# ZPP-Robotics/OSQP-Solver

Measured on AMD Instinct MI355X. Metric: QPs/sec on a 1024-QP batch of box-QPs (n=512, m=1024), OSQP defaults; ADMM iters/sec alongside, higher is better.
Workload: dtype f64

## Files before the change

### include/mi_osqp.h

```cpp
#ifndef MI_OSQP_H
#define MI_OSQP_H

#include <stdint.h>

#ifdef __cplusplus
extern "C" {
#endif

typedef enum {
  MI_OSQP_OK = 0,
  MI_OSQP_ERR_INVALID_DATA = 1,
  MI_OSQP_ERR_INVALID_SETTINGS = 2,
  MI_OSQP_ERR_PATTERN_CHANGED = 3,
  MI_OSQP_ERR_NONCONVEX = 4,
  MI_OSQP_ERR_DEVICE = 5,
  MI_OSQP_ERR_NULL = 6,
  MI_OSQP_ERR_ALLOC = 7
} mi_osqp_error;

typedef enum {
  MI_OSQP_EXIT_OPTIMAL = 0,
  MI_OSQP_EXIT_PRIMAL_INFEASIBLE = 1,
  MI_OSQP_EXIT_DUAL_INFEASIBLE = 2,
  MI_OSQP_EXIT_OPTIMAL_INACCURATE = 3,
// ... 112 lines not shown
                                  const double *l, const double *u);
int mi_osqp_batch_warm_start_x(mi_osqp_batch *h, const double *x);
int mi_osqp_batch_update_q(mi_osqp_batch *h, const double *q);
int mi_osqp_batch_update_P(mi_osqp_batch *h, const int64_t *P_colptr, const int64_t *P_rowidx, const double *P_val);
int mi_osqp_batch_update_P_A(mi_osqp_batch *h, const int64_t *P_colptr, const int64_t *P_rowidx, const double *P_val,
                             const int64_t *A_colptr, const int64_t *A_rowidx, const double *A_val);
int mi_osqp_batch_warm_start_y(mi_osqp_batch *h, const double *y);
int mi_osqp_batch_get_P_upper_pattern(mi_osqp_batch *h, int64_t *colptr, int64_t *rowidx, int64_t *nnz_out);
int mi_osqp_batch_solve(mi_osqp_batch *h);
int mi_osqp_batch_get_primal(mi_osqp_batch *h, double *x_out );
int mi_osqp_batch_get_dual(mi_osqp_batch *h, double *y_out );
int mi_osqp_batch_get_info(mi_osqp_batch *h, mi_osqp_info *info );
int mi_osqp_batch_get_prim_inf_cert(mi_osqp_batch *h, double *dy_out );
int mi_osqp_batch_get_dual_inf_cert(mi_osqp_batch *h, double *dx_out );
int mi_osqp_batch_get_stats(mi_osqp_batch *h, mi_osqp_stats *st);
int mi_osqp_batch_get_ordering(mi_osqp_batch *h, int64_t *kkt_perm);
void mi_osqp_batch_free(mi_osqp_batch *h);
int mi_osqp_prefetch_analysis(int64_t B, int64_t n, int64_t m, const int64_t *Pp, const int64_t *Pi,
                              const int64_t *Ap, const int64_t *Ai, int64_t device);
void mi_osqp_release_device_cache(void);

int mi_osqp_batch_update_bounds_device(mi_osqp_batch *h, const double *d_l, const double *d_u, void *stream);
int mi_osqp_batch_update_A_bounds_device(mi_osqp_batch *h, const double *d_Av, const double *d_l, const double *d_u, void *stream);
int mi_osqp_batch_update_q_device(mi_osqp_batch *h, const double *d_q, void *stream);
int mi_osqp_batch_update_P_device(mi_osqp_batch *h, const double *d_Pv, void *stream);
int mi_osqp_batch_update_P_A_bounds_device(mi_osqp_batch *h, const double *d_Pv, const double *d_Av, const double *d_l, const double *d_u,
                                           void *stream);
int mi_osqp_batch_solve_device(mi_osqp_batch *h, double *d_x_out, int32_t *d_status, int32_t *d_iters, void *stream);
int mi_osqp_batch_reset(mi_osqp_batch *h);
int mi_osqp_batch_last_solve_stats(mi_osqp_batch *h, int64_t *total_iters, int64_t *kernel_launches,
// ... 184 lines not shown
```

### osqp-solver_amd/__init__.py

```python
import ctypes as C
import os

import numpy as np

try:
    import torch
except ImportError:
    torch = None

from . import build as _build

_HERE = os.path.dirname(os.path.abspath(__file__))
_LIB = None

EXIT_NAMES = ["kOptimal", "kPrimalInfeasible", "kDualInfeasible", "kOptimalInaccurate",
              "kPrimalInfeasibleInaccurate", "kDualInfeasibleInaccurate", "kMaxIterations",
              "kInterrupted", "kTimeLimitReached", "kNonConvex", "kUnknown"]
K_OPTIMAL = 0


class Settings(C.Structure):
    _fields_ = [("rho", C.c_double), ("sigma", C.c_double), ("scaling", C.c_int64),
                ("adaptive_rho", C.c_int64), ("adaptive_rho_interval", C.c_int64),
                ("adaptive_rho_tolerance", C.c_double), ("max_iter", C.c_int64),
# ... 88 lines not shown
        L.mi_osqp_get_settings.argtypes = [vp, C.POINTER(Settings)]
        L.mi_osqp_update_settings.argtypes = [vp, C.POINTER(Settings)]
        L.mi_osqp_multi_batch_get_settings.argtypes = [vp, C.POINTER(Settings)]
        L.mi_osqp_multi_batch_update_settings.argtypes = [vp, C.POINTER(Settings)]
        L.mi_osqp_multi_batch_update_rho_each.argtypes = [vp, dp]
        L.mi_osqp_batch_solve.argtypes = [vp]
        L.mi_osqp_batch_get_primal.argtypes = [vp, dp]
        L.mi_osqp_batch_get_dual.argtypes = [vp, dp]
        L.mi_osqp_batch_get_info.argtypes = [vp, C.POINTER(Info)]
        for f in ("mi_osqp_get_prim_inf_cert", "mi_osqp_get_dual_inf_cert", "mi_osqp_batch_get_prim_inf_cert",
                  "mi_osqp_batch_get_dual_inf_cert", "mi_osqp_multi_batch_get_prim_inf_cert", "mi_osqp_multi_batch_get_dual_inf_cert"):
            getattr(L, f).argtypes = [vp, dp]
        L.mi_osqp_batch_get_prim_inf_cert_some.argtypes = [vp, C.c_int64, ip, dp]
        L.mi_osqp_batch_get_dual_inf_cert_some.argtypes = [vp, C.c_int64, ip, dp]
        L.mi_osqp_batch_get_stats.argtypes = [vp, C.POINTER(Stats)]
        L.mi_osqp_batch_get_ordering.argtypes = [vp, ip]
        L.mi_osqp_batch_free.argtypes = [vp]; L.mi_osqp_batch_free.restype = None
        L.mi_osqp_batch_update_bounds_device.argtypes = [vp, vp, vp, vp]
        L.mi_osqp_batch_update_A_bounds_device.argtypes = [vp, vp, vp, vp, vp]
        L.mi_osqp_batch_solve_device.argtypes = [vp, vp, vp, vp, vp]
        L.mi_osqp_batch_reset.argtypes = [vp]
        L.mi_osqp_batch_refactor_device.argtypes = [vp]
        L.mi_osqp_batch_last_solve_stats.argtypes = [vp, ip, ip, dp, dp, ip, dp]
        L.mi_osqp_batch_last_polish_stats.argtypes = [vp, ip, ip, dp]
        L.mi_osqp_batch_get_polish_active.argtypes = [vp, C.POINTER(C.c_int8)]
        L.mi_osqp_batch_adjoint.argtypes = [vp, dp, dp, dp, dp, dp, dp, dp, C.POINTER(C.c_int32)]
        L.mi_osqp_adjoint.argtypes = [vp, dp, dp, dp, dp, dp, dp, dp, C.POINTER(C.c_int32)]
        L.mi_osqp_batch_adjoint_device.argtypes = [vp] * 10
        L.mi_osqp_batch_get_scaling.argtypes = [vp, dp, dp, dp]
        L.mi_osqp_batch_spmv.argtypes = [vp, vp, vp, vp, vp, vp, vp]
# ... 212 lines not shown
    def prim_inf_cert(self):
        v = np.empty((self.B, self.m))
        _chk(lib().mi_osqp_batch_get_prim_inf_cert(self._h, _dp(v)), "get_prim_inf_cert")
        return v

    def dual_inf_cert(self):
        v = np.empty((self.B, self.n))
        _chk(lib().mi_osqp_batch_get_dual_inf_cert(self._h, _dp(v)), "get_dual_inf_cert")
        return v

    def stats(self):
        s = Stats()
        _chk(lib().mi_osqp_batch_get_stats(self._h, C.byref(s)), "get_stats")
        return s.as_dict()

    def ordering(self):
        perm = np.empty(self.n + self.m, dtype=np.int64)
        _chk(lib().mi_osqp_batch_get_ordering(self._h, _ip(perm)), "get_ordering")
        return perm

    def update_A(self, Ax, A_pattern=None):
        Ax = _f64(Ax).reshape(self.B, -1)
        Ap, Ai = self._Ap, self._Ai
        if A_pattern is not None:
            A = _csc(A_pattern)
            Ap, Ai = _i64(A.indptr), _i64(A.indices)
            if len(Ai) != len(self._Ai):
                raise MiOsqpError(3, "update_A")
        _chk(lib().mi_osqp_batch_update_A(self._h, _ip(Ap), _ip(Ai), _dp(Ax)), "update_A")

# ... 522 lines not shown
```

### osqp-solver_amd/csrc/device_types.h

```cpp
#pragma once
#include <hip/hip_runtime.h>
#include <stdint.h>

namespace miosqp {

#define MI_CHUNK 16

struct SchedDev {
  const uint32_t *step, *idxw;
  const uint64_t *idxw64;
  const uint32_t *lvl_pos, *tail_bar;
  int n_phases, nw, n_levels;
  uint32_t n_steps, n_slots;
};

struct DenseTailDev {
  int s, k, n_phases;
  uint32_t n_steps;
  const uint32_t *task;
  const uint32_t *wave_task, *wave_step, *tail_bar;
};

enum { DS_C = 0, DS_CINV, DS_RHO, DS_RHO_EST, DS_PRI_RES, DS_DUA_RES, DS_OBJ, DS_COUNT };
enum { IS_STATUS = 0, IS_ITER, IS_RHO_UPDATES, IS_DONE, IS_NEED_REFACTOR, IS_CUR, IS_PENDING, IS_EPOCH, IS_COUNT };
// ... 26 lines not shown
  int wide;
  double sigma, alpha, eps_abs, eps_rel, eps_prim_inf, eps_dual_inf, rho_tolerance;
  int check_termination, rho_interval, max_iter, scaled_termination, scaling, adaptive_rho;
  int iter_begin, iter_end;
  int op_out_lds;
  int info_at_end;
  int mw_groups;
  unsigned *mw_bar;
  double *mw_scratch;
  int df;
  unsigned df_shadow;
  const unsigned char *rflag;
  const int *sel;
  const int *tiles;
  double *res;
};

struct FactorArgs {
  int n, m, N, B, nnzP, nnzK, pa_len, n_levels, force_all;
  int debug_skip;
  uint32_t storage;
  SchedDev fwd, bwd;
  const uint32_t *blk, *lvl, *utask, *tri4, *dtask, *ttask, *asm_dst, *asm_src;
  const uint32_t *ubig;
  int *use_work;
  const int32_t *fwd_srcblk, *bwd_srcblk;
  const double *pa_val, *l, *u, *dscal;
  double *rho_vec, *rho_inv, *Lblk, *Dl, *dinv_scratch, *fwd_val, *bwd_val, *dinv;
  int *iscal, *npos;
  int home_bt;
// ... 163 lines not shown
```

### osqp-solver_amd/csrc/host_core.cpp

```cpp
#include "host_core.hpp"
#include "sched_format.h"

#include <algorithm>
#include <cmath>
#include <cstdio>
#include <cstdlib>
#include <cstring>
#include <limits>
#include <numeric>
#include <set>
#include <chrono>
#include <thread>

#include "../../include/mi_osqp.h"

namespace miosqp {

int validate_settings(const Settings &s) {
  if (s.scaling < 0 || s.max_iter <= 0 || s.check_termination < 0) return 1;
  if (s.adaptive_rho != 0 && s.adaptive_rho != 1) return 1;
  if (s.adaptive_rho_interval < 0 || s.adaptive_rho_tolerance < 1.0) return 1;
  if (!(s.rho > 0.0) || !(s.sigma > 0.0)) return 1;
  if (s.eps_abs < 0.0 || s.eps_rel < 0.0 || (s.eps_abs == 0.0 && s.eps_rel == 0.0)) return 1;
  if (!(s.eps_prim_inf > 0.0) || !(s.eps_dual_inf > 0.0)) return 1;
// ... 920 lines not shown
  t.stream_factor = getenv("MI_OSQP_STREAM_FACTOR") != nullptr;
  if (const char *e = getenv("MI_OSQP_REFACTOR_PIPELINE")) t.refactor_pipeline = atoi(e) != 0;
  if (const char *e = getenv("MI_OSQP_REFACTOR_PIPELINE_MIN")) t.pipeline_min = std::max(0, atoi(e));
  if (const char *e = getenv("MI_OSQP_REFACTOR_CHUNKS")) t.pipeline_chunks = std::max(0, std::min(8, atoi(e)));
  if (const char *e = getenv("MI_OSQP_REFACTOR_CHUNK_QPS")) t.pipeline_chunk_qps = std::max(0, atoi(e));
  if (const char *e = getenv("MI_OSQP_REFACTOR_LANES")) t.refactor_lanes = std::max(1, std::min(3, atoi(e)));
  if (const char *e = getenv("MI_OSQP_REFACTOR_CHUNK0")) t.lanes_chunk0 = atoi(e) != 0;
  if (const char *e = getenv("MI_OSQP_REGION_PRIORITY")) t.region_priority = std::max(0, std::min(2, atoi(e)));
  if (const char *e = getenv("MI_OSQP_LANE_CHECKS")) t.lane_checks = atoi(e) != 0;
  if (const char *e = getenv("MI_OSQP_RUNAHEAD")) t.runahead = atoi(e) != 0;
  if (const char *e = getenv("MI_OSQP_RUNAHEAD_TILES")) t.runahead_tiles = std::max(0, atoi(e));
  if (const char *e = getenv("MI_OSQP_RUNAHEAD_MIN")) t.runahead_min = std::max(0, atoi(e));
  if (const char *e = getenv("MI_OSQP_RUNAHEAD_END")) t.runahead_end = std::max(0, atoi(e));
  if (const char *e = getenv("MI_OSQP_RF_FORM")) { const int v = atoi(e); if (v == kIterDeepRing || v == kIterLongHead) t.rf_form = v; }
  if (const char *e = getenv("MI_OSQP_RF_LONG_MIN")) t.rf_long_min = std::max(0, atoi(e));
  if (const char *e = getenv("MI_OSQP_INDEX_LOADS")) t.index_loads = atoi(e) != 0;
  AnalysisTuning &a = t.analysis;
  if (const char *e = getenv("MI_OSQP_DENSE_TAIL")) a.dense_tail = atoi(e);
  if (const char *e = getenv("MI_OSQP_ORDERING")) a.ordering = e[0];
  if (const char *e = getenv("MI_OSQP_ND_LEAF")) a.nd_leaf = atoi(e);
  if (const char *e = getenv("MI_OSQP_RELAX")) a.relax = atoi(e);
  a.serial = getenv("MI_OSQP_SERIAL_ANALYSIS") != nullptr;
  return t;
}

RefactorChunks refactor_chunks(const std::vector<int> &flagged, const std::vector<int> &active, int bt, int chunk_qps, int max_chunks) {
  RefactorChunks rc;
  const int nq = (int)flagged.size();
  max_chunks = std::max(1, max_chunks);
  chunk_qps = std::max(1, chunk_qps);
// ... 899 lines not shown
```

### osqp-solver_amd/csrc/host_core.hpp

```cpp
#pragma once

#include <cstdint>
#include <string>
#include <vector>

namespace miosqp {

constexpr double kInfty = 1e30;
constexpr double kRhoMin = 1e-6, kRhoMax = 1e6, kRhoEqOverIneq = 1e3, kRhoTol = 1e-4;
constexpr double kMinScaling = 1e-4, kMaxScaling = 1e4;
constexpr double kDivisionTol = 1.0 / kInfty;
constexpr int kChunk = 16;
constexpr uint32_t kNoRow = 0xFFFFFFFFu;

struct Settings {
  double rho = 0.1, sigma = 1e-6;
  int64_t scaling = 10, adaptive_rho = 1, adaptive_rho_interval = 0;
  double adaptive_rho_tolerance = 5.0;
  int64_t max_iter = 4000;
  double eps_abs = 1e-3, eps_rel = 1e-3, eps_prim_inf = 1e-4, eps_dual_inf = 1e-4, alpha = 1.6;
  int64_t scaled_termination = 0, check_termination = 25, warm_start = 1, verbose = 0;
  int64_t polish = 0, polish_refine_iter = 3;
  double delta = 1e-6;
};
// ... 28 lines not shown
  bool stream_factor = false;
  bool refactor_pipeline = true;
  int pipeline_min = 0;
  int pipeline_chunks = 0;
  int pipeline_chunk_qps = 0;
  int refactor_lanes = 0;
  int lanes_chunk0 = -1;
  int region_priority = kRegionPriorityDefault;
  bool lane_checks = kLaneChecksDefault;
  bool runahead = kRunaheadDefault;
  int runahead_tiles = 0;
  int runahead_min = 0;
  int runahead_end = 0;
  int rf_form = 0;
  int rf_long_min = -1;
  bool index_loads = false;
  AnalysisTuning analysis;
};
Tuning tuning_from_env();

bool index_words_fit(bool resident_state, bool lds_vector, int bt, int threads, int64_t n, int64_t m);

enum IterateForm { kIterStreamed = 0, kIterDeepRing = 1, kIterLongHead = 2 };
constexpr int kRfLongMinDefault = 0;
int iterate_form(int tiles, bool has_head, const Tuning &t);

struct RefactorChunks {
  int n_chunks = 1;
  std::vector<int> work_begin;
  std::vector<int> tiles;
// ... 164 lines not shown
```

### osqp-solver_amd/csrc/kernels.hip

```cpp
#include <hip/hip_runtime.h>
#include <stdint.h>
#include <stdlib.h>
#include <string.h>

#include <algorithm>
#include <map>
#include <mutex>

#include "device_types.h"
#include "sched_format.h"

namespace miosqp {

static hipError_t ensure_dynamic_lds(const void *kern, size_t lds);

#define MI_INFTY 1e30
#define MI_MIN_SCALING 1e-4
#define MI_DIV_TOL 1e-30
#define MI_RHO_EST_DIV 1e-10
#define MI_RHO_MIN 1e-6
#define MI_RHO_MAX 1e6
#define MI_NOROW 0xFFFFFFFFu
#ifdef MI_OSQP_DEBUG_BUILD
#define MI_DBG_SKIP(a) ((a).debug_skip)
// ... 1035 lines not shown
          } else { zn = zp[u]; yn = yv[u]; }
          if (df) { st_sc1(xs + pos[u], zn - ri[u] * yn); df_arm_fwd(xs, (uint32_t)pos[u], fl[u], xl[u], sh); }
          else xs[pos[u]] = zn - ri[u] * yn;
        }
      }
    }
    if constexpr (GX) wg_or_grid_barrier(mw); else __syncthreads();
  }
}
template <int BT, int NT, bool GX, bool WIDE = false, bool RS = false, int RF = 0, bool IX = false>
__global__ __launch_bounds__(NT) void iterate_kernel(KernelArgs a) {
  extern __shared__ double smem[];
  iterate_body<BT, NT, GX, WIDE, RS, RF, IX>(a, smem, a.iter_end - a.iter_begin);
}

template <int BT, int NT, bool GX, bool WIDE = false>
__device__ __forceinline__ int check_body(const KernelArgs &a, double *smem, int n_iter) {
  bool dfm = false;
  if constexpr (GX && BT == 1 && WIDE) dfm = a.df != 0 && a.mw_groups > 1;
  const Mw mw{a.mw_bar, dfm ? (unsigned)a.mw_groups : 1u};
  const int tile = dfm ? 0 : (a.tiles ? a.tiles[blockIdx.x] : (int)blockIdx.x);
  const int ltid = threadIdx.x, lwave = __builtin_amdgcn_readfirstlane(ltid >> 6), lnw = blockDim.x >> 6;
  const int tid = dfm ? blockIdx.x * blockDim.x + threadIdx.x : threadIdx.x, nthr = dfm ? blockDim.x * mw.G : blockDim.x;
  const int lane = tid & 63, wave = __builtin_amdgcn_readfirstlane(tid >> 6), nw = nthr >> 6;
  const int b = tid % BT;
  auto sync = [&]() { if constexpr (GX && BT == 1 && WIDE) wg_or_grid_barrier(mw); else __syncthreads(); };
  auto gscratch = [&](int slot) { return a.mw_scratch + (size_t)slot * 256 * 16; };
  const int n = a.n, m = a.m;
  double *red;
  double *xs = solve_vector<BT, GX>(a, smem, tile, red);
  const TilePtrs<BT> p = tile_ptrs<BT>(a, tile, true);
// ... 2 lines not shown
  const int iter = p.iscal[IS_CUR * BT + b] + n_iter;
  int status = p.iscal[IS_STATUS * BT + b];
  int rho_updates = p.iscal[IS_RHO_UPDATES * BT + b];
  double rho = p.dscal[DS_RHO * BT + b];
  const double c = p.dscal[DS_C * BT + b], cinv = p.dscal[DS_CINV * BT + b];
  const bool unscale = a.scaling && !a.scaled_termination;
  const bool is_last = iter >= a.max_iter;
  const bool is_check = a.check_termination && (iter % a.check_termination == 0);
  const bool is_rho = a.adaptive_rho && a.rho_interval && (iter % a.rho_interval == 0);
  bool any_check = is_check || is_last, any_last = is_last;
  if constexpr (BT > 1) { any_check = __syncthreads_or(any_check); any_last = __syncthreads_or(any_last); }
  int need_refactor = 0;
  for (int e = tid; e < n * BT; e += nthr) xs[e] = p.x[e];
  for (int e = tid; e < m * BT; e += nthr) xs[(size_t)n * BT + e] = p.y[e];
  sync();
  run_spmv<BT, MI_PFV, WIDE>(a.chk, p.vchk, xs, p.out1, wave, lane, 0, 3, nw);
  sync();
  double mx[14];
#pragma unroll
  for (int k = 0; k < 14; k++) mx[k] = 0.0;
  double sm[1] = {0.0};
  for (int e = tid; e < n * BT; e += nthr) {
    const double px = p.out1[e], aty = p.out1[(size_t)n * BT + e], qv = p.q[e], xv = p.x[e];
    const double di = p.Dsc_inv[e];
    double dres = qv + px;
    dres += aty;
    mx[0] = fmax(mx[0], fabs(dres));      mx[1] = fmax(mx[1], fabs(di * dres));
    mx[2] = fmax(mx[2], fabs(qv));        mx[3] = fmax(mx[3], fabs(aty));   mx[4] = fmax(mx[4], fabs(px));
    mx[5] = fmax(mx[5], fabs(di * qv));   mx[6] = fmax(mx[6], fabs(di * aty)); mx[7] = fmax(mx[7], fabs(di * px));
    sm[0] += 0.5 * xv * px + qv * xv;
  }
  for (int e = tid; e < m * BT; e += nthr) {
    const double ax = p.out1[(size_t)2 * n * BT + e], zv = p.z[e], ei = p.Esc_inv[e];
    const double pres = ax - zv;
    mx[8] = fmax(mx[8], fabs(pres));      mx[9] = fmax(mx[9], fabs(ei * pres));
    mx[10] = fmax(mx[10], fabs(zv));      mx[11] = fmax(mx[11], fabs(ax));
    mx[12] = fmax(mx[12], fabs(ei * zv)); mx[13] = fmax(mx[13], fabs(ei * ax));
  }
  block_reduce<BT, 14, true>(mx, red, ltid, lwave, lnw, lane);
  block_reduce<BT, 1, false>(sm, red, ltid, lwave, lnw, lane);
  if constexpr (GX && BT == 1 && WIDE) {
    grid_reduce<14, true>(mx, red, mw, gscratch(0), ltid, lwave, lnw, lane);
    grid_reduce<1, false>(sm, red, mw, gscratch(1), ltid, lwave, lnw, lane);
  }
  const double pri_res = (m == 0) ? 0.0 : (unscale ? mx[9] : mx[8]);
  const double dua_res = unscale ? cinv * mx[1] : mx[0];
  double obj = sm[0];
  if (a.scaling) obj *= cinv;
  const double pri_nrm = unscale ? fmax(mx[12], mx[13]) : fmax(mx[10], mx[11]);
  const double dua_nrm = unscale ? cinv * fmax(fmax(mx[5], mx[6]), mx[7]) : fmax(fmax(mx[2], mx[3]), mx[4]);

  double mi[4] = {0.0, 0.0, 0.0, 0.0};
  double si[2] = {0.0, 0.0};
  for (int e = tid; e < n * BT; e += nthr) {
    const double d = p.dx[e];
    xs[e] = d;
    mi[1] = fmax(mi[1], unscale ? fabs(p.Dsc[e] * d) : fabs(d));
    si[1] += p.q[e] * d;
  }
  for (int e = tid; e < m * BT; e += nthr) {
    double d = p.dy[e];
    const double lo = p.l[e], up = p.u[e];
    if (up > MI_INFTY * MI_MIN_SCALING) {
      if (lo < -MI_INFTY * MI_MIN_SCALING) d = 0.0; else d = fmin(d, 0.0);
    } else if (lo < -MI_INFTY * MI_MIN_SCALING) d = fmax(d, 0.0);
    xs[(size_t)n * BT + e] = d;
    mi[0] = fmax(mi[0], unscale ? fabs(p.Esc[e] * d) : fabs(d));
    si[0] += up * fmax(d, 0.0) + lo * fmin(d, 0.0);
  }
  sync();
  run_spmv<BT, MI_PFV, WIDE>(a.chk, p.vchk, xs, p.out2, wave, lane, 0, 3, nw);
  sync();
  for (int e = tid; e < n * BT; e += nthr) {
    const double pdx = p.out2[e], atdy = p.out2[(size_t)n * BT + e];
    const double di = unscale ? p.Dsc_inv[e] : 1.0;
    mi[2] = fmax(mi[2], fabs(di * atdy));
    mi[3] = fmax(mi[3], fabs(di * pdx));
  }
  block_reduce<BT, 4, true>(mi, red, ltid, lwave, lnw, lane);
  block_reduce<BT, 2, false>(si, red, ltid, lwave, lnw, lane);
  if constexpr (GX && BT == 1 && WIDE) {
    grid_reduce<4, true>(mi, red, mw, gscratch(2), ltid, lwave, lnw, lane);
    grid_reduce<2, false>(si, red, mw, gscratch(3), ltid, lwave, lnw, lane);
  }
  const double norm_dy = mi[0], norm_dx = mi[1];
  const double cost_scaling = unscale ? c : 1.0;

  auto decide = [&](bool approx) -> int {
    const double f = approx ? 10.0 : 1.0;
    const double eps_abs = f * a.eps_abs, eps_rel = f * a.eps_rel;
    const double eps_pinf = f * a.eps_prim_inf, eps_dinf = f * a.eps_dual_inf;
    double viol[1] = {0.0};
    for (int e = tid; e < m * BT; e += nthr) {
      double adx = p.out2[(size_t)2 * n * BT + e];
      if (unscale) adx *= p.Esc_inv[e];
      const double lo = p.l[e], up = p.u[e];
      if ((up < MI_INFTY * MI_MIN_SCALING && adx > eps_dinf * norm_dx) ||
          (lo > -MI_INFTY * MI_MIN_SCALING && adx < -eps_dinf * norm_dx)) viol[0] = 1.0;
    }
    block_reduce<BT, 1, true>(viol, red, ltid, lwave, lnw, lane);
    if constexpr (GX && BT == 1 && WIDE) grid_reduce<1, true>(viol, red, mw, gscratch(approx ? 5 : 4), ltid, lwave, lnw, lane);
    if (pri_res > MI_INFTY || dua_res > MI_INFTY) return -7;
    int prim_ok = 0, dual_ok = 0, prim_inf = 0, dual_inf = 0;
    if (m == 0) prim_ok = 1;
    else {
      const double eps_prim = eps_abs + eps_rel * pri_nrm;
      if (pri_res < eps_prim) prim_ok = 1;
      else if (norm_dy > MI_DIV_TOL && si[0] < -eps_pinf * norm_dy) prim_inf = mi[2] < eps_pinf * norm_dy;
    }
    const double eps_dual = eps_abs + eps_rel * dua_nrm;
    if (dua_res < eps_dual) dual_ok = 1;
    else if (norm_dx > MI_DIV_TOL && si[1] < -cost_scaling * eps_dinf * norm_dx &&
             mi[3] < cost_scaling * eps_dinf * norm_dx) dual_inf = viol[0] == 0.0;
    if (prim_ok && dual_ok) return approx ? 2 : 1;
    if (prim_inf) return approx ? 3 : -3;
    if (dual_inf) return approx ? 4 : -4;
    return 0;
  };

  int new_status = 0;
  if (any_check) { const int s0 = decide(false); if (is_check || is_last) new_status = s0; }
  double rho_est = p.dscal[DS_RHO_EST * BT + b];
  auto rho_estimate = [&]() -> double {
    const double pr = mx[8] / (fmax(mx[10], mx[11]) + MI_RHO_EST_DIV);
    const double du = mx[0] / (fmax(fmax(mx[2], mx[3]), mx[4]) + MI_RHO_EST_DIV);
    double e = rho * sqrt(pr / du);
    return fmin(fmax(e, MI_RHO_MIN), MI_RHO_MAX);
  };
// ... 62 lines not shown
  if (tid < BT) {
    p.iscal[IS_DONE * BT + b] = done; p.iscal[IS_STATUS * BT + b] = status;
    p.iscal[IS_RHO_UPDATES * BT + b] = rho_updates;
    if (!was_done) { p.iscal[IS_NEED_REFACTOR * BT + b] = need_refactor; p.iscal[IS_CUR * BT + b] = iter; }
    p.dscal[DS_RHO * BT + b] = rho;
    if (a.res && !done && qp >= 0) { a.res[2 * (size_t)qp] = pri_res; a.res[2 * (size_t)qp + 1] = dua_res; }
  }
  int ev = (just_done ? 1 : 0) | (need_refactor ? 2 : 0);
  if constexpr (BT > 1) ev = (__syncthreads_or(ev & 1) ? 1 : 0) | (__syncthreads_or(ev & 2) ? 2 : 0);
  return ev;
}
template <int BT, int NT, bool GX, bool WIDE = false>
__global__ __launch_bounds__(NT) void check_kernel(KernelArgs a) {
  extern __shared__ double smem[];
  (void)check_body<BT, NT, GX, WIDE>(a, smem, a.iter_end - a.iter_begin);
}

struct AdvanceArgs {
  int max_segments, seg_len;
  int *host_is;
  double *host_ds;
  unsigned *stop;
  unsigned seq;
  unsigned *counter;
  unsigned *host_done;
};
template <int BT, int NT, bool RS = false>
__global__ __launch_bounds__(NT) void advance_kernel(KernelArgs a, AdvanceArgs v) {
  extern __shared__ double smem[];
  const int tile = blockIdx.x, tid = threadIdx.x;
// ... 2568 lines not shown
      if (a.rf_form == RF_FORM_DEEP_RING)
        return a.ix ? go(&iterate_kernel<1, 1024, false, false, true, RF_FORM_DEEP_RING, true>) : go(&iterate_kernel<1, 1024, false, false, true, RF_FORM_DEEP_RING>);
      return hipErrorInvalidValue;
    }
    if (a.ix) return BT == 1 ? go(&iterate_kernel<1, 1024, false, false, true, 0, true>) : go(&iterate_kernel<2, 1024, false, false, true, 0, true>);
    return BT == 1 ? go(&iterate_kernel<1, 1024, false, false, true>) : go(&iterate_kernel<2, 1024, false, false, true>);
  }
  if (a.rf_off || a.ix) return hipErrorInvalidValue;
  MI_DISPATCH(iterate_kernel, a);
}
hipError_t launch_check(const KernelArgs &a, int BT, int tiles, int threads, size_t lds, hipStream_t st) {
  if (!grid_form(a, BT, tiles, true, true)) return hipErrorInvalidValue;
#ifdef MI_OSQP_DEBUG_BUILD
  if (a.df && a.mw_groups > 1 && debug_drop_group("check") && tiles > 1) tiles--;
#endif
  MI_DISPATCH(check_kernel, a);
}
hipError_t launch_spmv(const KernelArgs &a, int BT, int tiles, int threads, size_t lds, hipStream_t st,
                       const double *x, const double *y, double *Px, double *Aty, double *Ax) {
  MI_DISPATCH(spmv_kernel, a, x, y, Px, Aty, Ax);
}
hipError_t launch_kkt_solve(const KernelArgs &a, int BT, int tiles, int threads, size_t lds, hipStream_t st,
                            const double *rhs, double *sol) {
  if (!grid_form(a, BT, tiles, false, false)) return hipErrorInvalidValue;
#ifdef MI_OSQP_DEBUG_BUILD
  if (a.df && debug_drop_group("kkt") && tiles > 1) tiles--;
#endif
  MI_DISPATCH(kkt_solve_kernel, a, rhs, sol);
}
hipError_t launch_polish_active(const KernelArgs &a, const PolishArgs &p, int BT, hipStream_t st) {
// ... 92 lines not shown
```

### osqp-solver_amd/csrc/solver.hip

```cpp
#include <hip/hip_runtime.h>
#include <time.h>

#include <algorithm>
#include <atomic>
#include <chrono>
#include <cmath>
#include <condition_variable>
#include <functional>
#include <limits>
#include <cstdio>
#include <cstdlib>
#include <cstring>
#include <string>
#include <thread>
#include <map>
#include <memory>
#include <mutex>
#include <vector>

#include "../../include/mi_osqp.h"
#include "device_types.h"
#include "host_core.hpp"
#include "sched_format.h"

// ... 238 lines not shown
  int ix = 0;
  int64_t rf_launches[3] = {0, 0, 0};
  std::vector<QPNumeric> qp;
  bool host_bounds_stale = false;
  hipStream_t stream = nullptr;
  SchedBufs fwd, bwd, chk;
  DevBuf<uint32_t> pinv, xloc;
  DevBuf<double> fwd_val, bwd_val, chk_val, dinv, x, z, y, q, l, u, rho_vec, rho_inv, Dsc, Dsc_inv, Esc, Esc_inv;
  DevBuf<double> dx, dy, out1, out2, dscal, x_out, y_out, xs_global;
  DevBuf<double> cert_out;
  bool global_xs = false;
  int mw_groups = 0, mw_threads = 0;
  DevBuf<uint32_t> mw_bar;
  DevBuf<unsigned char> rflag;
  DevBuf<double> mw_scratch;
  DevBuf<double> fwd_val0, bwd_val0, dinv0, rho_vec0, rho_inv0, dscal0;
  DevBuf<int> use_work;
  DevBuf<int> iscal, flag, npos;
  DevBuf<uint32_t> bf_blk, bf_lvl, bf_utask, bf_tri, bf_dtask, bf_ttask, bf_asm_dst, bf_asm_src, bf_ubig;
  DevBuf<int32_t> fwd_srcblk, bwd_srcblk;
  DevBuf<double> pa_val, Lblk, Dl, dinv_scratch;
  DevBuf<uint32_t> dt_task, dt_wave_task, dt_wave_step, dt_tail_bar;
  DevBuf<uint32_t> dt_lt_pos, dt_ltcol_col, dt_tile_tab, dt_wave_tiles, dt_diag_tile, dt_task_step;
  DevBuf<uint64_t> dt_asm_q64;
  DevBuf<int32_t> dt_src_tile;
  int dt_nh = 0; uint32_t dt_cs_doubles = 0; size_t dt_lds = 0, dt_lds_asm = 0;
  DevBuf<int32_t> dt_src;
  DevBuf<double> dt_val, dt_val0, dt_Sd;
  DevBuf<uint32_t> sp_ptr, sp_ent;
  DevBuf<uint32_t> sp_ell, sp_rowid;
// ... 143 lines not shown
  a.rf_form = iterate_form(h->ntiles, h->rf_off != 0, h->tune);
  a.mw_groups = h->mw_groups; a.mw_bar = h->mw_bar.p; a.mw_scratch = h->mw_scratch.p;
  a.df = (*h->anp).df ? 1 : 0; a.df_shadow = (unsigned)(*h->anp).Next; a.rflag = h->rflag.p;
  {
    const DenseTail &dt = (*h->anp).dt;
    a.dt.s = dt.s; a.dt.k = dt.k; a.dt.n_phases = dt.n_phases; a.dt.n_steps = dt.n_steps;
    a.dt.task = h->dt_task.p; a.dt.wave_task = h->dt_wave_task.p; a.dt.wave_step = h->dt_wave_step.p; a.dt.tail_bar = h->dt_tail_bar.p;
    a.dt_val = h->dt_val.p;
  }
  const Settings &s = h->st;
  a.sigma = s.sigma; a.alpha = s.alpha; a.eps_abs = s.eps_abs; a.eps_rel = s.eps_rel;
  a.eps_prim_inf = s.eps_prim_inf; a.eps_dual_inf = s.eps_dual_inf; a.rho_tolerance = s.adaptive_rho_tolerance;
  a.check_termination = (int)s.check_termination; a.rho_interval = (int)s.adaptive_rho_interval;
  a.max_iter = (int)s.max_iter; a.scaled_termination = (int)s.scaled_termination; a.scaling = s.scaling ? 1 : 0;
  a.adaptive_rho = (int)s.adaptive_rho; a.iter_begin = 0; a.iter_end = 0; a.info_at_end = 1;
  return a;
}

static FactorArgs make_factor_args(mi_osqp_batch *h, int force_all) {
  FactorArgs a{};
  const Analysis &an = (*h->anp);
  a.n = an.n; a.m = an.m; a.N = an.N; a.B = h->B; a.nnzP = an.Pp[an.n]; a.nnzK = an.nnzK();
  a.pa_len = an.Pp[an.n] + an.Ap[an.n]; a.n_levels = an.bf.n_levels; a.force_all = force_all;
  a.storage = an.bf.storage; a.fwd = h->fwd.view(an.fwd); a.bwd = h->bwd.view(an.bwd);
  a.blk = h->bf_blk.p; a.lvl = h->bf_lvl.p; a.utask = h->bf_utask.p; a.tri4 = h->bf_tri.p; a.dtask = h->bf_dtask.p; a.ubig = h->bf_ubig.p;
  a.ttask = h->bf_ttask.p; a.asm_dst = h->bf_asm_dst.p; a.asm_src = h->bf_asm_src.p;
  a.fwd_srcblk = h->fwd_srcblk.p; a.bwd_srcblk = h->bwd_srcblk.p;
  a.pa_val = h->pa_val.p; a.l = h->l.p; a.u = h->u.p; a.dscal = h->dscal.p;
  a.rho_vec = h->rho_vec.p; a.rho_inv = h->rho_inv.p; a.Lblk = h->Lblk.p; a.Dl = h->Dl.p; a.dinv_scratch = h->dinv_scratch.p;
  a.fwd_val = h->fwd_val.p; a.bwd_val = h->bwd_val.p; a.dinv = h->dinv.p; a.iscal = h->iscal.p; a.npos = h->npos.p; a.use_work = h->use_work.p;
// ... 408 lines not shown
  { std::vector<uint32_t> pv(an.pinv.begin(), an.pinv.end()); if ((rc = h->pinv.upload(pv))) return rc; }
  { std::vector<uint32_t> xv(an.xloc.begin(), an.xloc.end()); if ((rc = h->xloc.upload(xv))) return rc; }
  {
    std::vector<int32_t> pr(an.Pi.begin(), an.Pi.begin() + an.Pp[n]), pc(an.Pp[n]), ar(an.Ai.begin(), an.Ai.begin() + an.Ap[n]), ac(an.Ap[n]);
    for (int j = 0; j < n; j++) { for (int k = an.Pp[j]; k < an.Pp[j + 1]; k++) pc[k] = j; for (int k = an.Ap[j]; k < an.Ap[j + 1]; k++) ac[k] = j; }
    if ((rc = h->rz_prow.upload(pr)) || (rc = h->rz_pcol.upload(pc)) || (rc = h->rz_arow.upload(ar)) || (rc = h->rz_acol.upload(ac))) return rc;
  }
  if ((rc = h->use_work.alloc(T)) || (rc = h->use_work.zero(h->stream))) return rc;
#define ALLOC(buf, len) if ((rc = h->buf.alloc((size_t)(len) * T)) || (rc = h->buf.zero(h->stream))) return rc
  ALLOC(fwd_val, (size_t)an.fwd.phys_steps() * 64); ALLOC(bwd_val, (size_t)an.bwd.phys_steps() * 64); ALLOC(chk_val, (size_t)an.chk.phys_steps() * 64); ALLOC(dinv, an.N);
  ALLOC(x, n); ALLOC(z, m); ALLOC(y, m); ALLOC(q, n); ALLOC(l, m); ALLOC(u, m); ALLOC(rho_vec, m); ALLOC(rho_inv, m);
  ALLOC(Dsc, n); ALLOC(Dsc_inv, n); ALLOC(Esc, m); ALLOC(Esc_inv, m); ALLOC(dx, n); ALLOC(dy, m);
  ALLOC(out1, 2 * n + m); ALLOC(out2, 2 * n + m); ALLOC(dscal, DS_COUNT);
  if (h->global_xs) { ALLOC(xs_global, an.xs_total); }
  if ((rc = h->mw_bar.alloc(4 * (size_t)std::max(h->n_cus, 1))) || (rc = h->mw_bar.zero(h->stream))) return rc;
  if (an.df && ((rc = h->rflag.upload(an.rflag)) || (rc = h->mw_scratch.alloc((size_t)8 * 256 * 16)) || (rc = h->mw_scratch.zero(h->stream)))) return rc;
  if (an.dt.k) {
    const DenseTail &dt = an.dt;
    ALLOC(dt_val, (size_t)dt.n_steps * 64);
    if ((rc = h->dt_task.upload(dt.task)) || (rc = h->dt_wave_task.upload(dt.wave_task)) || (rc = h->dt_wave_step.upload(dt.wave_step)) ||
        (rc = h->dt_tail_bar.upload(dt.tail_bar)) || (rc = h->dt_src.upload(dt.src)) ||
        (rc = h->dt_lt_pos.upload(dt.lt_pos)) || (rc = h->dt_ltcol_col.upload(dt.ltcol_col)) || (rc = h->dt_tile_tab.upload(dt.tile_tab)) ||
        (rc = h->dt_wave_tiles.upload(dt.wave_tiles)) || (rc = h->dt_asm_q64.upload(dt.asm_q64)) ||
        (rc = h->dt_src_tile.upload(dt.src_tile)) || (rc = h->dt_diag_tile.upload(dt.diag_tile)) || (rc = h->dt_task_step.upload(dt.task_step)) ||
        (rc = h->dt_Sd.alloc((size_t)dt.k * dt.k * (T + 4)))) return rc;
    const int nrt = dt.k / 16 - 4;
    h->dt_nh = nrt <= 14 ? std::max(nrt, 1) : (nrt + 1) / 2;
    h->dt_cs_doubles = (uint32_t)std::max(h->dt_nh * 1024, 64 * 65 + 63) / 64 * 64;
    h->dt_lds = std::max<size_t>((size_t)h->dt_cs_doubles + 4096, 2 * 64 * 65) * sizeof(double);
    h->dt_lds_asm = (dt.asm_lds_bytes() + 255) & ~(size_t)255;
// ... 1071 lines not shown
}

int mi_osqp_batch_get_stats(mi_osqp_batch *h, mi_osqp_stats *st) {
  if (!h || !st) return MI_OSQP_ERR_NULL;
  *st = h->stats;
  st->pipelined_refactors = h->pipelined_refactors;
  st->refactor_lanes = h->refactor_lanes;
  st->iterate_launches_deep_ring = h->rf_launches[RF_FORM_DEEP_RING];
  st->iterate_launches_long_head = h->rf_launches[RF_FORM_LONG_HEAD];
  st->runahead_regions = h->ra_regions; st->runahead_tiles = h->ra_tiles;
  st->runahead_left = h->ra_left; st->runahead_missed = h->ra_missed;
  st->region_priority = h->region_priority; st->region_lane_checks = h->region_lane_checks; st->region_chunks = h->region_chunks;
  return MI_OSQP_OK;
}

int mi_osqp_batch_get_ordering(mi_osqp_batch *h, int64_t *kkt_perm) {
  if (!h || !kkt_perm) return MI_OSQP_ERR_NULL;
  const Analysis &an = (*h->anp);
  for (int k = 0; k < an.N; k++) kkt_perm[k] = an.perm[(size_t)k];
  return MI_OSQP_OK;
}

int mi_osqp_batch_last_solve_stats(mi_osqp_batch *h, int64_t *total_iters, int64_t *kernel_launches, double *device_seconds,
                                   double *refactor_seconds, int64_t *refactor_count, double *compact_seconds) {
  if (!h) return MI_OSQP_ERR_NULL;
  if (compact_seconds) *compact_seconds = 0.0;
  if (total_iters) *total_iters = h->last_total_iters;
  if (kernel_launches) *kernel_launches = h->last_launches;
  if (device_seconds) *device_seconds = h->last_device_s;
  if (refactor_seconds) *refactor_seconds = h->last_refactor_s;
// ... 2325 lines not shown
```

Baseline: 46750.

## Skip infeasibility SpMV in termination check unless pretests flag infeasibility

The termination check kernel now evaluates convergence and the cheap infeasibility pretests first. It runs the second SpMV on (dx, dy) and the violation scan only when a certificate test could fire, with an env override to force the full path. When occupancy allows, a new LDS variant keeps the first SpMV output in shared memory rather than global memory. Every check also does a global atomic counter increment for diagnostics, which adds a small cost and extra host logic to choose the kernel variant.

```diff
diff --git a/include/mi_osqp.h b/include/mi_osqp.h
--- a/include/mi_osqp.h
+++ b/include/mi_osqp.h
@@ -150,6 +150,7 @@
 int mi_osqp_batch_get_prim_inf_cert(mi_osqp_batch *h, double *dy_out );
 int mi_osqp_batch_get_dual_inf_cert(mi_osqp_batch *h, double *dx_out );
 int mi_osqp_batch_get_stats(mi_osqp_batch *h, mi_osqp_stats *st);
+int mi_osqp_batch_check_counts(mi_osqp_batch *h, int64_t *tile_checks, int64_t *with_products);
 int mi_osqp_batch_get_ordering(mi_osqp_batch *h, int64_t *kkt_perm);
 void mi_osqp_batch_free(mi_osqp_batch *h);
 int mi_osqp_prefetch_analysis(int64_t B, int64_t n, int64_t m, const int64_t *Pp, const int64_t *Pi,
diff --git a/osqp-solver_amd/__init__.py b/osqp-solver_amd/__init__.py
--- a/osqp-solver_amd/__init__.py
+++ b/osqp-solver_amd/__init__.py
@@ -126,6 +126,7 @@
         L.mi_osqp_batch_get_prim_inf_cert_some.argtypes = [vp, C.c_int64, ip, dp]
         L.mi_osqp_batch_get_dual_inf_cert_some.argtypes = [vp, C.c_int64, ip, dp]
         L.mi_osqp_batch_get_stats.argtypes = [vp, C.POINTER(Stats)]
+        L.mi_osqp_batch_check_counts.argtypes = [vp, ip, ip]
         L.mi_osqp_batch_get_ordering.argtypes = [vp, ip]
         L.mi_osqp_batch_free.argtypes = [vp]; L.mi_osqp_batch_free.restype = None
         L.mi_osqp_batch_update_bounds_device.argtypes = [vp, vp, vp, vp]
@@ -368,6 +369,11 @@
         _chk(lib().mi_osqp_batch_get_stats(self._h, C.byref(s)), "get_stats")
         return s.as_dict()
 
+    def check_counts(self):
+        tc, wp = C.c_int64(), C.c_int64()
+        _chk(lib().mi_osqp_batch_check_counts(self._h, C.byref(tc), C.byref(wp)), "check_counts")
+        return dict(tile_checks=tc.value, with_products=wp.value)
+
     def ordering(self):
         perm = np.empty(self.n + self.m, dtype=np.int64)
         _chk(lib().mi_osqp_batch_get_ordering(self._h, _ip(perm)), "get_ordering")
diff --git a/osqp-solver_amd/csrc/device_types.h b/osqp-solver_amd/csrc/device_types.h
--- a/osqp-solver_amd/csrc/device_types.h
+++ b/osqp-solver_amd/csrc/device_types.h
@@ -64,6 +64,9 @@
   const int *sel;
   const int *tiles;
   double *res;
+  int chk_full;
+  unsigned long long *chk_count;
+  int chk_out_off;
 };
 
 struct FactorArgs {
diff --git a/osqp-solver_amd/csrc/host_core.cpp b/osqp-solver_amd/csrc/host_core.cpp
--- a/osqp-solver_amd/csrc/host_core.cpp
+++ b/osqp-solver_amd/csrc/host_core.cpp
@@ -958,6 +958,7 @@
   if (const char *e = getenv("MI_OSQP_RUNAHEAD_END")) t.runahead_end = std::max(0, atoi(e));
   if (const char *e = getenv("MI_OSQP_RF_FORM")) { const int v = atoi(e); if (v == kIterDeepRing || v == kIterLongHead) t.rf_form = v; }
   if (const char *e = getenv("MI_OSQP_RF_LONG_MIN")) t.rf_long_min = std::max(0, atoi(e));
+  if (const char *e = getenv("MI_OSQP_CHECK_FULL")) t.check_full = atoi(e) != 0;
   if (const char *e = getenv("MI_OSQP_INDEX_LOADS")) t.index_loads = atoi(e) != 0;
   AnalysisTuning &a = t.analysis;
   if (const char *e = getenv("MI_OSQP_DENSE_TAIL")) a.dense_tail = atoi(e);
diff --git a/osqp-solver_amd/csrc/host_core.hpp b/osqp-solver_amd/csrc/host_core.hpp
--- a/osqp-solver_amd/csrc/host_core.hpp
+++ b/osqp-solver_amd/csrc/host_core.hpp
@@ -66,6 +66,7 @@
   int runahead_end = 0;
   int rf_form = 0;
   int rf_long_min = -1;
+  bool check_full = false;
   bool index_loads = false;
   AnalysisTuning analysis;
 };
diff --git a/osqp-solver_amd/csrc/kernels.hip b/osqp-solver_amd/csrc/kernels.hip
--- a/osqp-solver_amd/csrc/kernels.hip
+++ b/osqp-solver_amd/csrc/kernels.hip
@@ -1073,7 +1073,7 @@
   iterate_body<BT, NT, GX, WIDE, RS, RF, IX>(a, smem, a.iter_end - a.iter_begin);
 }
 
-template <int BT, int NT, bool GX, bool WIDE = false>
+template <int BT, int NT, bool GX, bool WIDE = false, bool O1L = false>
 __device__ __forceinline__ int check_body(const KernelArgs &a, double *smem, int n_iter) {
   bool dfm = false;
   if constexpr (GX && BT == 1 && WIDE) dfm = a.df != 0 && a.mw_groups > 1;
@@ -1106,14 +1106,16 @@
   for (int e = tid; e < n * BT; e += nthr) xs[e] = p.x[e];
   for (int e = tid; e < m * BT; e += nthr) xs[(size_t)n * BT + e] = p.y[e];
   sync();
-  run_spmv<BT, MI_PFV, WIDE>(a.chk, p.vchk, xs, p.out1, wave, lane, 0, 3, nw);
+  double *o1;
+  if constexpr (O1L) o1 = smem + a.chk_out_off; else o1 = p.out1;
+  run_spmv<BT, MI_PFV, WIDE>(a.chk, p.vchk, xs, o1, wave, lane, 0, 3, nw);
   sync();
   double mx[14];
 #pragma unroll
   for (int k = 0; k < 14; k++) mx[k] = 0.0;
   double sm[1] = {0.0};
   for (int e = tid; e < n * BT; e += nthr) {
-    const double px = p.out1[e], aty = p.out1[(size_t)n * BT + e], qv = p.q[e], xv = p.x[e];
+    const double px = o1[e], aty = o1[(size_t)n * BT + e], qv = p.q[e], xv = p.x[e];
     const double di = p.Dsc_inv[e];
     double dres = qv + px;
     dres += aty;
@@ -1123,7 +1125,7 @@
     sm[0] += 0.5 * xv * px + qv * xv;
   }
   for (int e = tid; e < m * BT; e += nthr) {
-    const double ax = p.out1[(size_t)2 * n * BT + e], zv = p.z[e], ei = p.Esc_inv[e];
+    const double ax = o1[(size_t)2 * n * BT + e], zv = p.z[e], ei = p.Esc_inv[e];
     const double pres = ax - zv;
     mx[8] = fmax(mx[8], fabs(pres));      mx[9] = fmax(mx[9], fabs(ei * pres));
     mx[10] = fmax(mx[10], fabs(zv));      mx[11] = fmax(mx[11], fabs(ax));
@@ -1142,7 +1144,7 @@
   const double pri_nrm = unscale ? fmax(mx[12], mx[13]) : fmax(mx[10], mx[11]);
   const double dua_nrm = unscale ? cinv * fmax(fmax(mx[5], mx[6]), mx[7]) : fmax(fmax(mx[2], mx[3]), mx[4]);
 
-  double mi[4] = {0.0, 0.0, 0.0, 0.0};
+  double mi[2] = {0.0, 0.0};
   double si[2] = {0.0, 0.0};
   for (int e = tid; e < n * BT; e += nthr) {
     const double d = p.dx[e];
@@ -1160,50 +1162,73 @@
     mi[0] = fmax(mi[0], unscale ? fabs(p.Esc[e] * d) : fabs(d));
     si[0] += up * fmax(d, 0.0) + lo * fmin(d, 0.0);
   }
-  sync();
-  run_spmv<BT, MI_PFV, WIDE>(a.chk, p.vchk, xs, p.out2, wave, lane, 0, 3, nw);
-  sync();
-  for (int e = tid; e < n * BT; e += nthr) {
-    const double pdx = p.out2[e], atdy = p.out2[(size_t)n * BT + e];
-    const double di = unscale ? p.Dsc_inv[e] : 1.0;
-    mi[2] = fmax(mi[2], fabs(di * atdy));
-    mi[3] = fmax(mi[3], fabs(di * pdx));
-  }
-  block_reduce<BT, 4, true>(mi, red, ltid, lwave, lnw, lane);
+  block_reduce<BT, 2, true>(mi, red, ltid, lwave, lnw, lane);
   block_reduce<BT, 2, false>(si, red, ltid, lwave, lnw, lane);
   if constexpr (GX && BT == 1 && WIDE) {
-    grid_reduce<4, true>(mi, red, mw, gscratch(2), ltid, lwave, lnw, lane);
+    grid_reduce<2, true>(mi, red, mw, gscratch(2), ltid, lwave, lnw, lane);
     grid_reduce<2, false>(si, red, mw, gscratch(3), ltid, lwave, lnw, lane);
   }
   const double norm_dy = mi[0], norm_dx = mi[1];
   const double cost_scaling = unscale ? c : 1.0;
 
+  auto pretest = [&](double f) -> int {
+    const double eps_abs = f * a.eps_abs, eps_rel = f * a.eps_rel;
+    const double eps_pinf = f * a.eps_prim_inf, eps_dinf = f * a.eps_dual_inf;
+    int r = 0;
+    if (m == 0) r |= 1;
+    else {
+      const double eps_prim = eps_abs + eps_rel * pri_nrm;
+      if (pri_res < eps_prim) r |= 1;
+      else if (norm_dy > MI_DIV_TOL && si[0] < -eps_pinf * norm_dy) r |= 4;
+    }
+    const double eps_dual = eps_abs + eps_rel * dua_nrm;
+    if (dua_res < eps_dual) r |= 2;
+    else if (norm_dx > MI_DIV_TOL && si[1] < -cost_scaling * eps_dinf * norm_dx) r |= 8;
+    return r;
+  };
+  const int pre_exact = pretest(1.0), pre_approx = pretest(10.0);
+  bool products = !done && (is_check || is_last) && (pre_exact & 12);
+  if (a.chk_full) products = true;
+  if constexpr (BT > 1) products = __syncthreads_or(products);
+  if (a.chk_count && tid == 0) __hip_atomic_fetch_add(a.chk_count + (products ? 1 : 0), 1ull, __ATOMIC_RELAXED, __HIP_MEMORY_SCOPE_AGENT);
+  double mp[2] = {0.0, 0.0};
+  if (products) {
+    sync();
+    run_spmv<BT, MI_PFV, WIDE>(a.chk, p.vchk, xs, p.out2, wave, lane, 0, 3, nw);
+    sync();
+    for (int e = tid; e < n * BT; e += nthr) {
+      const double pdx = p.out2[e], atdy = p.out2[(size_t)n * BT + e];
+      const double di = unscale ? p.Dsc_inv[e] : 1.0;
+      mp[0] = fmax(mp[0], fabs(di * atdy));
+      mp[1] = fmax(mp[1], fabs(di * pdx));
+    }
+    block_reduce<BT, 2, true>(mp, red, ltid, lwave, lnw, lane);
+    if constexpr (GX && BT == 1 && WIDE) grid_reduce<2, true>(mp, red, mw, gscratch(6), ltid, lwave, lnw, lane);
+  }
+
   auto decide = [&](bool approx) -> int {
     const double f = approx ? 10.0 : 1.0;
-    const double eps_abs = f * a.eps_abs, eps_rel = f * a.eps_rel;
     const double eps_pinf = f * a.eps_prim_inf, eps_dinf = f * a.eps_dual_inf;
+    const int pre = approx ? pre_approx : pre_exact;
     double viol[1] = {0.0};
-    for (int e = tid; e < m * BT; e += nthr) {
-      double adx = p.out2[(size_t)2 * n * BT + e];
-      if (unscale) adx *= p.Esc_inv[e];
-      const double lo = p.l[e], up = p.u[e];
-      if ((up < MI_INFTY * MI_MIN_SCALING && adx > eps_dinf * norm_dx) ||
-          (lo > -MI_INFTY * MI_MIN_SCALING && adx < -eps_dinf * norm_dx)) viol[0] = 1.0;
-    }
-    block_reduce<BT, 1, true>(viol, red, ltid, lwave, lnw, lane);
-    if constexpr (GX && BT == 1 && WIDE) grid_reduce<1, true>(viol, red, mw, gscratch(approx ? 5 : 4), ltid, lwave, lnw, lane);
+    if (products) {
+      for (int e = tid; e < m * BT; e += nthr) {
+        double adx = p.out2[(size_t)2 * n * BT + e];
+        if (unscale) adx *= p.Esc_inv[e];
+        const double lo = p.l[e], up = p.u[e];
+        if ((up < MI_INFTY * MI_MIN_SCALING && adx > eps_dinf * norm_dx) ||
+            (lo > -MI_INFTY * MI_MIN_SCALING && adx < -eps_dinf * norm_dx)) viol[0] = 1.0;
+      }
+      block_reduce<BT, 1, true>(viol, red, ltid, lwave, lnw, lane);
+      if constexpr (GX && BT == 1 && WIDE) grid_reduce<1, true>(viol, red, mw, gscratch(approx ? 5 : 4), ltid, lwave, lnw, lane);
+    }
     if (pri_res > MI_INFTY || dua_res > MI_INFTY) return -7;
-    int prim_ok = 0, dual_ok = 0, prim_inf = 0, dual_inf = 0;
-    if (m == 0) prim_ok = 1;
-    else {
-      const double eps_prim = eps_abs + eps_rel * pri_nrm;
-      if (pri_res < eps_prim) prim_ok = 1;
-      else if (norm_dy > MI_DIV_TOL && si[0] < -eps_pinf * norm_dy) prim_inf = mi[2] < eps_pinf * norm_dy;
-    }
-    const double eps_dual = eps_abs + eps_rel * dua_nrm;
-    if (dua_res < eps_dual) dual_ok = 1;
-    else if (norm_dx > MI_DIV_TOL && si[1] < -cost_scaling * eps_dinf * norm_dx &&
-             mi[3] < cost_scaling * eps_dinf * norm_dx) dual_inf = viol[0] == 0.0;
+    const int prim_ok = pre & 1, dual_ok = pre & 2;
+    int prim_inf = 0, dual_inf = 0;
+    if (products) {
+      if (pre & 4) prim_inf = mp[0] < eps_pinf * norm_dy;
+      if ((pre & 8) && mp[1] < cost_scaling * eps_dinf * norm_dx) dual_inf = viol[0] == 0.0;
+    }
     if (prim_ok && dual_ok) return approx ? 2 : 1;
     if (prim_inf) return approx ? 3 : -3;
     if (dual_inf) return approx ? 4 : -4;
@@ -1296,6 +1321,11 @@
 __global__ __launch_bounds__(NT) void check_kernel(KernelArgs a) {
   extern __shared__ double smem[];
   (void)check_body<BT, NT, GX, WIDE>(a, smem, a.iter_end - a.iter_begin);
+}
+template <int BT, int NT>
+__global__ __launch_bounds__(NT) void check_lds_kernel(KernelArgs a) {
+  extern __shared__ double smem[];
+  (void)check_body<BT, NT, false, false, true>(a, smem, a.iter_end - a.iter_begin);
 }
 
 struct AdvanceArgs {
@@ -3894,6 +3924,39 @@
 #ifdef MI_OSQP_DEBUG_BUILD
   if (a.df && a.mw_groups > 1 && debug_drop_group("check") && tiles > 1) tiles--;
 #endif
+  if (!a.chk_full && !a.xs_global && !a.wide && !a.df && threads <= 1024 && (threads > 512 ? BT <= 2 : BT <= 4)) {
+    const size_t lds_o1 = lds + (size_t)(2 * a.n + a.m) * BT * sizeof(double);
+    auto pick = [&](auto kg, auto kl) -> hipError_t {
+      static std::mutex mu;
+      static std::map<std::pair<int, size_t>, bool> fits;
+      bool ok;
+      {
+        std::lock_guard<std::mutex> lock(mu);
+        auto it = fits.find({threads, lds_o1});
+        if (it == fits.end()) {
+          int ng = 0, nl = 0;
+          ok = lds_o1 <= 160 * 1024 && ensure_dynamic_lds(reinterpret_cast<const void *>(kg), lds) == hipSuccess &&
+               ensure_dynamic_lds(reinterpret_cast<const void *>(kl), lds_o1) == hipSuccess &&
+               hipOccupancyMaxActiveBlocksPerMultiprocessor(&ng, reinterpret_cast<const void *>(kg), threads, lds) == hipSuccess &&
+               hipOccupancyMaxActiveBlocksPerMultiprocessor(&nl, reinterpret_cast<const void *>(kl), threads, lds_o1) == hipSuccess && nl >= ng && nl > 0;
+          (void)hipGetLastError();
+          it = fits.emplace(std::make_pair(threads, lds_o1), ok).first;
+        }
+        ok = it->second;
+      }
+      KernelArgs b = a;
+      b.chk_out_off = ok ? (int)(lds / sizeof(double)) : 0;
+      hipError_t e = ensure_dynamic_lds(ok ? reinterpret_cast<const void *>(kl) : reinterpret_cast<const void *>(kg), ok ? lds_o1 : lds);
+      if (e != hipSuccess) return e;
+      if (ok) hipLaunchKernelGGL(kl, dim3(tiles), dim3(threads), lds_o1, st, b);
+      else hipLaunchKernelGGL(kg, dim3(tiles), dim3(threads), lds, st, b);
+      return hipGetLastError();
+    };
+    if (threads > 512) return BT == 1 ? pick(&check_kernel<1, 1024, false>, &check_lds_kernel<1, 1024>) : pick(&check_kernel<2, 1024, false>, &check_lds_kernel<2, 1024>);
+    if (BT == 1) return pick(&check_kernel<1, 512, false>, &check_lds_kernel<1, 512>);
+    if (BT == 2) return pick(&check_kernel<2, 512, false>, &check_lds_kernel<2, 512>);
+    return pick(&check_kernel<4, 512, false>, &check_lds_kernel<4, 512>);
+  }
   MI_DISPATCH(check_kernel, a);
 }
 hipError_t launch_spmv(const KernelArgs &a, int BT, int tiles, int threads, size_t lds, hipStream_t st,
diff --git a/osqp-solver_amd/csrc/solver.hip b/osqp-solver_amd/csrc/solver.hip
--- a/osqp-solver_amd/csrc/solver.hip
+++ b/osqp-solver_amd/csrc/solver.hip
@@ -276,6 +276,7 @@
   DevBuf<uint32_t> mw_bar;
   DevBuf<unsigned char> rflag;
   DevBuf<double> mw_scratch;
+  DevBuf<unsigned long long> chk_count;
   DevBuf<double> fwd_val0, bwd_val0, dinv0, rho_vec0, rho_inv0, dscal0;
   DevBuf<int> use_work;
   DevBuf<int> iscal, flag, npos;
@@ -449,6 +450,7 @@
   a.check_termination = (int)s.check_termination; a.rho_interval = (int)s.adaptive_rho_interval;
   a.max_iter = (int)s.max_iter; a.scaled_termination = (int)s.scaled_termination; a.scaling = s.scaling ? 1 : 0;
   a.adaptive_rho = (int)s.adaptive_rho; a.iter_begin = 0; a.iter_end = 0; a.info_at_end = 1;
+  a.chk_full = h->tune.check_full ? 1 : 0; a.chk_count = h->chk_count.p;
   return a;
 }
 
@@ -887,6 +889,7 @@
   ALLOC(out1, 2 * n + m); ALLOC(out2, 2 * n + m); ALLOC(dscal, DS_COUNT);
   if (h->global_xs) { ALLOC(xs_global, an.xs_total); }
   if ((rc = h->mw_bar.alloc(4 * (size_t)std::max(h->n_cus, 1))) || (rc = h->mw_bar.zero(h->stream))) return rc;
+  if ((rc = h->chk_count.alloc(2)) || (rc = h->chk_count.zero(h->stream))) return rc;
   if (an.df && ((rc = h->rflag.upload(an.rflag)) || (rc = h->mw_scratch.alloc((size_t)8 * 256 * 16)) || (rc = h->mw_scratch.zero(h->stream)))) return rc;
   if (an.dt.k) {
     const DenseTail &dt = an.dt;
@@ -1988,6 +1991,17 @@
   return MI_OSQP_OK;
 }
 
+int mi_osqp_batch_check_counts(mi_osqp_batch *h, int64_t *tile_checks, int64_t *with_products) {
+  if (!h) return MI_OSQP_ERR_NULL;
+  DevGuard guard(h->device);
+  unsigned long long c[2] = {0, 0};
+  HIPCHK(hipStreamSynchronize(h->stream));
+  if (h->chk_count.p) HIPCHK(hipMemcpy(c, h->chk_count.p, sizeof(c), hipMemcpyDeviceToHost));
+  if (tile_checks) *tile_checks = (int64_t)(c[0] + c[1]);
+  if (with_products) *with_products = (int64_t)c[1];
+  return MI_OSQP_OK;
+}
+
 int mi_osqp_batch_get_ordering(mi_osqp_batch *h, int64_t *kkt_perm) {
   if (!h || !kkt_perm) return MI_OSQP_ERR_NULL;
   const Analysis &an = (*h->anp);
```

Result: no change. 47090 (median of 6 runs) (+0.7%).
